# lambdaclass/simpleworks

Hardware: AMD Instinct MI355X
Metric: Marlin prove() constraints/sec at 2^20 R1CS; G1 MSM points/sec (higher is better)
Workload: dtype u32 limbs (384-bit Montgomery Fq for G1, 256-bit Fr); 1 GPU; marlin_prove: synthetic R1CS, 2^20 constraints = variables = non-zeros per matrix (|H| = |K| = 2^20), SRS + proving key device resident; per_gpu_units=1048576, multi_gpu=replicas (one proof per rank)

## Files before the change

simpleworks_amd/_lib.py:

```python
import contextlib
import ctypes
import json
import os

import numpy as np

_HERE = os.path.dirname(os.path.abspath(__file__))
LIB_PATH = os.environ.get("SWM_LIB_PATH") or os.path.join(_HERE, "libswmarlin.so")

_u64p = ctypes.POINTER(ctypes.c_uint64)
_u32p = ctypes.POINTER(ctypes.c_uint32)
_vp = ctypes.c_void_p
_sz = ctypes.c_size_t
_int = ctypes.c_int

ABI = {
    "swm_version": (_int, []),
    "swm_strerror": (ctypes.c_char_p, [_int]),
    "swm_init": (_int, [_int, ctypes.POINTER(_vp)]),
    "swm_destroy": (None, [_vp]),
    "swm_last_error": (ctypes.c_char_p, [_vp]),
    "swm_set_stream": (_int, [_vp, _vp]),
    "swm_set_msm_sharding": (_int, [_vp, ctypes.c_uint, ctypes.c_uint, _vp, _vp]),
    "swm_rccl_unique_id": (_int, [ctypes.c_void_p]),
# ... 1127 lines not shown
        self._check(self.lib.swm_blake2s_witness(self.h, a.ctypes.data if a.size else None, a.shape[1], a.shape[0], witness.ctypes.data,
                                                 digests.ctypes.data), "swm_blake2s_witness")
        return witness, digests

    def blake2s_witness_dev(self, d_inputs, input_len, count, d_witness, d_digests=None):
        self._check(self.lib.swm_blake2s_witness_dev(self.h, self._dev_ptr(d_inputs), input_len, count, self._dev_ptr(d_witness),
                                                     self._dev_ptr(d_digests)), "swm_blake2s_witness_dev")

    def profile_enable(self, on=True):
        self._check(self.lib.swm_profile_enable(self.h, int(on)), "swm_profile_enable")

    def profile_reset(self):
        self._check(self.lib.swm_profile_reset(self.h), "swm_profile_reset")

    def profile(self):
        buf = ctypes.create_string_buffer(1 << 20)
        self._check(self.lib.swm_profile_json(self.h, buf, len(buf)), "swm_profile_json")
        doc = json.loads(buf.value.decode())
        self.last_work = doc.get("work", {})
        self.last_calls = doc.get("calls", [])
        return {k["name"]: k for k in doc["kernels"]}

    def selftest_mul(self, which, a, b):
        a = np.ascontiguousarray(a, dtype=np.uint64)
        b = np.ascontiguousarray(b, dtype=np.uint64)
        out = np.empty_like(a)
        self._check(self.lib.swm_selftest_mul(self.h, which, _p64(a), _p64(b), _p64(out), a.shape[0]), "swm_selftest_mul")
        return out

    def selftest_g1_add(self, a_xy, b_xy):
        a = np.ascontiguousarray(a_xy, dtype=np.uint64).reshape(-1, 12)
        b = np.ascontiguousarray(b_xy, dtype=np.uint64).reshape(-1, 12)
        out = np.zeros((a.shape[0], 18), dtype=np.uint64)
        self._check(self.lib.swm_selftest_g1_add(self.h, _p64(a), _p64(b), _p64(out), a.shape[0]), "swm_selftest_g1_add")
        return out

    G1_CODEC_OPS = {"encode": 0, "decode": 1, "decode_unchecked": 2}

    def selftest_g1_codec(self, op, data, n):
        bad = ctypes.c_uint(0)
        if op == "encode":
            a = np.ascontiguousarray(data, dtype=np.uint64).reshape(n, 12)
            out = np.zeros(n * 96, dtype=np.uint8)
            self._check(self.lib.swm_selftest_g1_codec(self.h, 0, a.ctypes.data, n, out.ctypes.data, None), "swm_selftest_g1_codec")
            return out.tobytes()
        a = np.frombuffer(bytes(data), dtype=np.uint8).copy()
        assert a.size == n * 96
        out = np.zeros((n, 12), dtype=np.uint64)
        self._check(self.lib.swm_selftest_g1_codec(self.h, self.G1_CODEC_OPS[op], a.ctypes.data, n, out.ctypes.data, ctypes.byref(bad)),
                    "swm_selftest_g1_codec")
        return out, bad.value

    FR29_OPS = {"mul": 0, "mul_c": 1, "normalize": 2, "cond_sub_2r": 3, "cond_sub_r": 4, "canonical_below_2r": 5,
                "canonical": 6, "sub": 7, "unpack": 8, "pack": 9, "inv": 10, "inv_exact": 11}

    def selftest_fr29(self, op, a9, b9=None, spread9=None):
        a = np.ascontiguousarray(a9, dtype=np.uint32).reshape(-1, 9)
        b = np.ascontiguousarray(b9 if b9 is not None else a, dtype=np.uint32).reshape(-1, 9)
        assert b.shape == a.shape
        sp = np.ascontiguousarray(spread9 if spread9 is not None else np.zeros(9), dtype=np.uint32).reshape(9)
        out = np.zeros_like(a)
        self._check(self.lib.swm_selftest_fr29(self.h, self.FR29_OPS[op], _p32(a), _p32(b), _p32(sp), _p32(out), a.shape[0]),
                    "swm_selftest_fr29")
        return out

    P28_OPS = {"dbl": 0, "add": 1, "add_ool": 2, "slot_add": 3, "slot_add_inplace": 4, "slot_dbl": 5, "store_384": 6, "madd28": 7,
               "rows": 8, "te_from_row": 9, "te_madd_row": 10, "te_slot_add": 11, "te_slot_add_inplace": 12, "te_slot_add_self": 13,
               "te_slot_add_sync": 14, "te_store_384": 15, "quad_from_row": 16, "quad_madd_row": 17, "quad_add": 18,
               "quad_add_self": 19, "quad_store_identity": 20}

    def selftest_p28(self, op, a, b=None, flags=None, backmap=False, n=None):
        if a is not None:
            a = np.ascontiguousarray(a, dtype=np.uint64).reshape(-1, 12 if op == "rows" else 24)
            n = a.shape[0]
        if n is None:
            raise ValueError("selftest_p28: an op without operand a needs n")
        if b is not None:
            b = np.ascontiguousarray(b, dtype=np.uint64).reshape(-1, 24)
            assert b.shape[0] == n
        if flags is not None:
            flags = np.ascontiguousarray(flags, dtype=np.uint32).reshape(-1)
            assert flags.shape[0] == n
        out = np.zeros((n, 24), dtype=np.uint64)
        status = np.zeros(max(n, 1), dtype=np.uint32)
        jac = np.zeros((n, 18), dtype=np.uint64) if backmap else None
        self._check(self.lib.swm_selftest_p28(self.h, self.P28_OPS[op], _p64(a) if a is not None else None,
                                              _p64(b) if b is not None else None, _p32(flags) if flags is not None else None,
                                              _p64(out), _p64(jac) if backmap else None, _p32(status), n), "swm_selftest_p28")
        return out, status[:n], jac

    def _poly(self, op, data, n, m, z, pieces, out):
        zz = np.ascontiguousarray(z if z is not None else np.zeros(4), dtype=np.uint64).reshape(4)
        pc = np.ascontiguousarray(pieces if pieces is not None else np.zeros(2), dtype=np.uint64).reshape(-1)
        self._check(self.lib.swm_selftest_poly(self.h, op, data.ctypes.data, n, m, _p64(zz), _p64(pc), pc.size // 2,
                                               out.ctypes.data if out is not None else None), "swm_selftest_poly")

    def selftest_suffix_recurrence(self, a_mont, m, z_mont):
        a = np.ascontiguousarray(a_mont, dtype=np.uint64).reshape(-1, 4).copy()
        self._poly(0, a, a.shape[0], m, z_mont, None, None)
        return a

    def selftest_div_linear(self, p_mont, z_mont):
        p = np.ascontiguousarray(p_mont, dtype=np.uint64).reshape(-1, 4)
        out = np.zeros_like(p)
        self._poly(1, p, p.shape[0], 0, z_mont, None, out)
        return out

# ... 93 lines not shown
```

simpleworks_amd/csrc/capi.hip:

```cpp
#include <dlfcn.h>
#include <stdarg.h>
#include <string.h>
#include <algorithm>
#include <vector>
#include "context.h"
#include "g1.cuh"
#include "msm.h"

struct swm_rccl_id_arg {
    char internal[128];
};

namespace swm {

int ntt_run(swm_ctx* ctx, void* d_data, unsigned log_n, int inverse, int coset);
int ntt_sharded_run(swm_ctx* ctx, void* d_local, unsigned log_n, int inverse, int blocks_in);
struct SpmvPlan;
int spmv_run(swm_ctx* ctx, const void* d_rowptr, const void* d_col, const void* d_val, const void* d_z, void* d_out,
             size_t rows, const SpmvPlan* plan = nullptr);
int vec_mul_run(swm_ctx* ctx, const void* a, const void* b, void* out, size_t n);
int batch_inverse_run(swm_ctx* ctx, void* d, size_t n);
int selftest_mul_run(swm_ctx* ctx, int which, const void* a, const void* b, void* out, size_t n);
int selftest_chain_run(swm_ctx* ctx, int which, void* out, size_t threads, int iters);
int selftest_g1_add_run(swm_ctx* ctx, const void* a, const void* b, void* out, size_t n);
// ... 792 lines not shown
    snprintf(tail, sizeof(tail),
             "],\"work\":{\"msm_calls\":%llu,\"msm_points\":%llu,\"msm_digits\":%llu,\"msm_adds\":%llu,\"msm_zero_points\":%llu,\"msm_twins\":%llu,\"ntt_calls\":%llu,"
             "\"ntt_elements\":%llu,\"spmv_calls\":%llu,\"spmv_rows\":%llu,\"spmv_nnz\":%llu}}",
             (unsigned long long)ctx->stat_msm_calls, (unsigned long long)ctx->stat_msm_points,
             (unsigned long long)ctx->stat_msm_digits, (unsigned long long)ctx->stat_msm_adds,
             (unsigned long long)ctx->stat_msm_zero_points, (unsigned long long)ctx->stat_msm_twins, (unsigned long long)ctx->stat_ntt_calls, (unsigned long long)ctx->stat_ntt_elems,
             (unsigned long long)ctx->stat_spmv_calls, (unsigned long long)ctx->stat_spmv_rows,
             (unsigned long long)ctx->stat_spmv_nnz);
    s += tail;
    s.pop_back();
    s += ",\"calls\":[";
    for (size_t i = 0; i < ctx->call_log.size(); i++) {
        char item[48];
        snprintf(item, sizeof(item), "%s[\"%c\",%llu]", i ? "," : "", ctx->call_log[i].first,
                 (unsigned long long)ctx->call_log[i].second);
        s += item;
    }
    s += "]}";
    if (s.size() + 1 > buflen) return set_err(ctx, SWM_ERR_INVALID_ARG, "profile_json: buffer too small");
    memcpy(buf, s.c_str(), s.size() + 1);
    return SWM_OK;
}

int swm_selftest_witness_stage(swm_ctx* ctx, size_t bytes) {
    if (!ctx) return SWM_ERR_INVALID_ARG;
    ctx->witness_stage_bytes = bytes ? bytes : WITNESS_STAGE_BYTES;
    return SWM_OK;
}
int swm_selftest_exchange(swm_ctx* ctx, const void* d_send, void* d_recv, size_t bytes_per_peer, int alltoall) {
    if (!ctx || !d_send || !d_recv) return SWM_ERR_INVALID_ARG;
    SWM_ON_DEVICE(ctx);
    if (alltoall) SWM_TRY(shard_alltoall_dev(ctx, d_send, d_recv, bytes_per_peer));
    else SWM_TRY(shard_allgather_dev(ctx, d_send, bytes_per_peer, d_recv));
    SWM_HIP(ctx, hipStreamSynchronize(ctx->stream));
    return SWM_OK;
}
int swm_selftest_mul(swm_ctx* ctx, int which, const uint64_t* a, const uint64_t* b, uint64_t* out, size_t n) {
    if (!ctx || !a || !b || !out) return SWM_ERR_INVALID_ARG;
    SWM_ON_DEVICE(ctx);
    size_t es = which == 1 ? 32 : 48;
    char *da = nullptr, *db = nullptr;
    SWM_TRY(scratch(ctx, "stage.a", n * es + 64, (void**)&da));
    SWM_TRY(scratch(ctx, "stage.b", n * es + 64, (void**)&db));
    SWM_HIP(ctx, hipMemcpyAsync(da, a, n * es, hipMemcpyHostToDevice, ctx->stream));
    SWM_HIP(ctx, hipMemcpyAsync(db, b, n * es, hipMemcpyHostToDevice, ctx->stream));
    SWM_TRY(selftest_mul_run(ctx, which, da, db, da, n));
    SWM_HIP(ctx, hipMemcpyAsync(out, da, n * es, hipMemcpyDeviceToHost, ctx->stream));
    SWM_HIP(ctx, hipStreamSynchronize(ctx->stream));
    return SWM_OK;
}
int swm_selftest_fr29(swm_ctx* ctx, int op, const uint32_t* a9, const uint32_t* b9, const uint32_t* spread9, uint32_t* out9,
                      size_t n) {
    const bool two = op == 0 || op == 1 || op == 7;
    if (!ctx || op < 0 || op > 11 || (n && (!a9 || !out9 || (two && !b9))) || (op == 7 && !spread9)) return SWM_ERR_INVALID_ARG;
    SWM_ON_DEVICE(ctx);
    if (n == 0) return SWM_OK;
    const size_t bytes = n * 36;
    char *da = nullptr, *db = nullptr;
    SWM_TRY(scratch(ctx, "stage.a", bytes + 64, (void**)&da));
    SWM_TRY(scratch(ctx, "stage.b", bytes + 64, (void**)&db));
    SWM_HIP(ctx, hipMemcpyAsync(da, a9, bytes, hipMemcpyHostToDevice, ctx->stream));
    if (two) SWM_HIP(ctx, hipMemcpyAsync(db, b9, bytes, hipMemcpyHostToDevice, ctx->stream));
    SWM_TRY(selftest_fr29_run(ctx, op, da, db, op == 7 ? spread9 : nullptr, da, n));
    SWM_HIP(ctx, hipMemcpyAsync(out9, da, bytes, hipMemcpyDeviceToHost, ctx->stream));
    SWM_HIP(ctx, hipStreamSynchronize(ctx->stream));
    return SWM_OK;
}
int swm_selftest_p28(swm_ctx* ctx, int op, const uint64_t* a, const uint64_t* b, const uint32_t* flags, uint64_t* out, uint64_t* out_jac,
                     uint32_t* status, size_t n) {
    const bool rows = op == 8, te = (op >= 9 && op <= 14) || (op >= 16 && op <= 20);
    const bool two = op == 1 || op == 2 || op == 3 || op == 4 || op == 7 || op == 10 || op == 11 || op == 12 || op == 14 || op == 17 || op == 18;
    if (!ctx || op < 0 || op > 20 || (n && (!out || (op != 20 && !a) || (two && !b))) || (out_jac && !te)) return SWM_ERR_INVALID_ARG;
    SWM_ON_DEVICE(ctx);
    if (n == 0) return SWM_OK;
    const size_t in_bytes = n * (rows ? 96 : 192), out_bytes = n * 192;
    char *da = nullptr, *db = nullptr, *dc = nullptr, *dd = nullptr;
    SWM_TRY(scratch(ctx, "stage.a", out_bytes + 64, (void**)&da));
    SWM_TRY(scratch(ctx, "stage.b", out_bytes + 64, (void**)&db));
    SWM_TRY(scratch(ctx, "stage.c", out_bytes + 64, (void**)&dc));
    SWM_TRY(scratch(ctx, "stage.d", n * 200 + 64, (void**)&dd));
    char* d_pref = dd + n * 144;
    uint32_t *d_flags = (uint32_t*)(dd + n * 192), *d_status = d_flags + n;
    if (a) SWM_HIP(ctx, hipMemcpyAsync(da, a, in_bytes, hipMemcpyHostToDevice, ctx->stream));
    if (two) SWM_HIP(ctx, hipMemcpyAsync(db, b, out_bytes, hipMemcpyHostToDevice, ctx->stream));
    if (flags) SWM_HIP(ctx, hipMemcpyAsync(d_flags, flags, n * 4, hipMemcpyHostToDevice, ctx->stream));
    else SWM_HIP(ctx, hipMemsetAsync(d_flags, 0, n * 4, ctx->stream));
    SWM_HIP(ctx, hipMemsetAsync(d_status, 0, n * 4, ctx->stream));
    SWM_HIP(ctx, hipMemsetAsync(dc, 0xA5, out_bytes, ctx->stream));
    SWM_TRY(selftest_p28_run(ctx, op, da, db, d_flags, dc, out_jac ? dd : nullptr, d_pref, d_status, n));
    SWM_HIP(ctx, hipMemcpyAsync(out, dc, out_bytes, hipMemcpyDeviceToHost, ctx->stream));
    if (out_jac) SWM_HIP(ctx, hipMemcpyAsync(out_jac, dd, n * 144, hipMemcpyDeviceToHost, ctx->stream));
    if (status) SWM_HIP(ctx, hipMemcpyAsync(status, d_status, n * 4, hipMemcpyDeviceToHost, ctx->stream));
    SWM_HIP(ctx, hipStreamSynchronize(ctx->stream));
    return SWM_OK;
}
int swm_selftest_g1_add(swm_ctx* ctx, const uint64_t* a_xy, const uint64_t* b_xy, uint64_t* out_jac, size_t n) {
    if (!ctx || !a_xy || !b_xy || !out_jac) return SWM_ERR_INVALID_ARG;
    SWM_ON_DEVICE(ctx);
    char *da = nullptr, *db = nullptr, *dc = nullptr;
    SWM_TRY(scratch(ctx, "stage.a", n * 96 + 64, (void**)&da));
    SWM_TRY(scratch(ctx, "stage.b", n * 96 + 64, (void**)&db));
    SWM_TRY(scratch(ctx, "stage.c", n * 144 + 64, (void**)&dc));
    SWM_HIP(ctx, hipMemcpyAsync(da, a_xy, n * 96, hipMemcpyHostToDevice, ctx->stream));
    SWM_HIP(ctx, hipMemcpyAsync(db, b_xy, n * 96, hipMemcpyHostToDevice, ctx->stream));
    SWM_TRY(selftest_g1_add_run(ctx, da, db, dc, n));
    SWM_HIP(ctx, hipMemcpyAsync(out_jac, dc, n * 144, hipMemcpyDeviceToHost, ctx->stream));
    SWM_HIP(ctx, hipStreamSynchronize(ctx->stream));
// ... 109 lines not shown
```

simpleworks_amd/csrc/fr29.cuh:

```cuda
#pragma once
#include "ff.cuh"

namespace swm {

struct Fr29 {
    uint32_t l[9];
};
static constexpr uint32_t M29 = (1u << 29) - 1;
struct Fr29Consts {
    static constexpr uint32_t P[9] = SWM_FR29_P;
    static constexpr uint32_t ONE[9] = SWM_FR29_ONE;
    static constexpr uint32_t P2[9] = SWM_FR29_2P;
};

__device__ __forceinline__ Fr29 fr29_unpack(const Fr& a) {
    Fr29 r;
#pragma unroll
    for (int i = 0; i < 9; i++) {
        const int bit = 29 * i, w = bit >> 5, off = bit & 31;
        uint32_t v = a.v[w] >> off;
        if (off > 3 && w + 1 < 8) v |= a.v[w + 1] << (32 - off);
        r.l[i] = i < 8 ? (v & M29) : v;
    }
    return r;
// ... 33 lines not shown
#pragma unroll
    for (int i = 0; i < 9; i++) r.l[i] = a.l[i] + b.l[i];
    return r;
}
struct Spread29 {
    uint32_t l[9];
};
__device__ __forceinline__ Fr29 fr29_sub(const Fr29& a, const Fr29& b, const Spread29& sp) {
    Fr29 r;
#pragma unroll
    for (int i = 0; i < 9; i++) r.l[i] = a.l[i] + sp.l[i] - b.l[i];
    return r;
}
__device__ __forceinline__ Fr29 fr29_mul(const Fr29& a, const Fr29& b) {
    Fr29 r;
    uint32_t m[9];
    uint64_t acc = 0;
#pragma unroll
    for (int k = 0; k < 9; k++) {
#pragma unroll
        for (int i = 0; i <= k; i++) acc += (uint64_t)a.l[i] * b.l[k - i];
#pragma unroll
        for (int i = 0; i < k; i++) acc += (uint64_t)m[i] * Fr29Consts::P[k - i];
        m[k] = (0u - (uint32_t)acc) & M29;
        acc = (acc + m[k]) >> 29;
    }
#pragma unroll
    for (int k = 9; k < 17; k++) {
#pragma unroll
        for (int i = k - 8; i < 9; i++) acc += (uint64_t)a.l[i] * b.l[k - i];
#pragma unroll
        for (int i = k - 8; i < 9; i++) acc += (uint64_t)m[i] * Fr29Consts::P[k - i];
        r.l[k - 9] = (uint32_t)acc & M29;
        acc >>= 29;
    }
    r.l[8] = (uint32_t)acc;
    return r;
}
#include "fr29_mul_asm.inc"
__device__ __forceinline__ Fr29 fr29_mul_fenced(const Fr29& a, const Fr29& b) {
    Fr29 r;
    uint32_t m0, m1, m2, m3, m4, m5, m6, m7, m8;
    constexpr const uint32_t (&P)[9] = Fr29Consts::P;
    static_assert(P[0] == 1u, "the carry rule needs r = 1 mod 2^29");
    asm(SWM_FR29_MUL_ASM_TEXT
        : "=&v"(r.l[0]), "=&v"(r.l[1]), "=&v"(r.l[2]), "=&v"(r.l[3]), "=&v"(r.l[4]), "=&v"(r.l[5]), "=&v"(r.l[6]), "=&v"(r.l[7]),
          "=&v"(r.l[8]), "=&v"(m0), "=&v"(m1), "=&v"(m2), "=&v"(m3), "=&v"(m4), "=&v"(m5), "=&v"(m6), "=&v"(m7), "=&v"(m8)
        : "v"(a.l[0]), "v"(a.l[1]), "v"(a.l[2]), "v"(a.l[3]), "v"(a.l[4]), "v"(a.l[5]), "v"(a.l[6]), "v"(a.l[7]), "v"(a.l[8]),
          "v"(b.l[0]), "v"(b.l[1]), "v"(b.l[2]), "v"(b.l[3]), "v"(b.l[4]), "v"(b.l[5]), "v"(b.l[6]), "v"(b.l[7]), "v"(b.l[8]),
          "s"(P[1]), "s"(P[2]), "s"(P[3]), "s"(P[4]), "s"(P[5]), "s"(P[6]), "s"(P[7]), "s"(P[8]), "s"(M29), "s"((uint64_t)M29)
        : "v0", "v1", "vcc");
    return r;
}
__device__ __forceinline__ Fr29 fr29_cond_sub(const Fr29& a, const uint32_t (&k)[9]) {
    Fr29 t;
    uint32_t borrow = 0;
#pragma unroll
    for (int i = 0; i < 9; i++) {
        uint32_t d = a.l[i] - k[i] - borrow;
        borrow = d >> 31;
        t.l[i] = i < 8 ? (d & M29) : d;
    }
    Fr29 r;
#pragma unroll
    for (int i = 0; i < 9; i++) r.l[i] = borrow ? a.l[i] : t.l[i];
    return r;
}
__device__ __forceinline__ Fr29 fr29_canonical(const Fr29& a, bool below_2r) {
    Fr29 x = below_2r ? a : fr29_cond_sub(a, Fr29Consts::P2);
    return fr29_cond_sub(x, Fr29Consts::P);
}

}
```

simpleworks_amd/csrc/ntt.hip:

```cpp
#include <atomic>
#include "context.h"
#include "ff.cuh"
#include "fr29.cuh"
#include <string.h>
#include <algorithm>
#include <vector>

namespace swm {

static constexpr int NTT_THREADS = 256;
static constexpr unsigned NTT_MAX_LOG_R = 10;

struct NttPassArgs {
    const Fr* src;
    Fr* dst;
    unsigned log_n, log_r, log_ns;
    const Fr* tw_small;
    const Fr* tw_lo;
    const Fr* tw_hi;
    const Fr* cs_lo;
    const Fr* cs_hi;
    uint64_t src_len;
    const Fr* pass_tw;
    int coset_in;
// ... 155 lines not shown
    const NttPassArgs& a = args.a;
    const LazyPlan& P = args.plan;
    const unsigned R = 1u << a.log_r;
    const uint64_t n = 1ull << a.log_n;
    const uint64_t stride = n >> a.log_r;
    const uint64_t j0 = (uint64_t)blockIdx.x * J;
    const uint64_t ns_mask = (1ull << a.log_ns) - 1;
    const unsigned tw_shift = a.log_n - a.log_ns - a.log_r;
    const Fr* src = a.src + blockIdx.y * a.src_cstride;
    Fr* dst = a.dst + blockIdx.y * a.dst_cstride;
    const uint64_t cs_k = a.cos_k[blockIdx.y];
    for (unsigned e0 = 0; e0 < R * J; e0 += 4 * NTT_THREADS) {
        Fr xs[4];
#pragma unroll
        for (int u = 0; u < 4; u++) {
            unsigned e = e0 + threadIdx.x + u * NTT_THREADS;
            if (e < R * J) {
                const uint64_t at = j0 + e % J + (uint64_t)(e / J) * stride;
                xs[u] = at < a.src_len ? src[at] : fp_zero<Fr>();
                if (a.fold_in && at + n < a.src_len) xs[u] = fp_add(xs[u], fp_mul(a.fold[blockIdx.y], src[at + n]));
            }
        }
#pragma unroll
        for (int u = 0; u < 4; u++) {
            unsigned e = e0 + threadIdx.x + u * NTT_THREADS;
            if (e >= R * J) break;
            unsigned jj = e % J, t = e / J;
            uint64_t idx = j0 + jj + (uint64_t)t * stride;
            Fr29 x = fr29_unpack(xs[u]);
            if (a.coset_in) x = fr29_mul_fenced(x, two_level_pow29(a.cs_lo, a.cs_hi, idx * cs_k));
            if (a.log_ns != 0) {
                uint64_t k = (j0 + jj) & ns_mask;
                const Fr29 tw = a.pass_tw ? fr29_unpack(a.pass_tw[((uint64_t)t << a.log_ns) + k])
                                          : two_level_pow29(a.tw_lo, a.tw_hi, (k * t) << tw_shift);
                x = fr29_mul_fenced(x, tw);
            }
            tile_put(tile, t * J + jj, x);
        }
    }
    __syncthreads();
    unsigned h = R >> 1;
    if (a.log_r & 1) {
        for (unsigned bq = threadIdx.x; bq < (R >> 1) * J; bq += NTT_THREADS) {
            unsigned jj = bq % J, pos = bq / J;
            unsigned i0 = pos, i1 = i0 + h;
            Fr29 u = tile_get(tile, i0 * J + jj), v = tile_get(tile, i1 * J + jj);
            tile_put(tile, i0 * J + jj, fr29_normalize(fr29_add(u, v)));
            tile_put(tile, i1 * J + jj, fr29_mul_fenced(fr29_sub(u, v, P.r2), fr29_unpack(a.tw_small[pos])));
        }
        h >>= 1;
        __syncthreads();
    }
    unsigned step = 0;
    for (; h >= 2; h >>= 2, step++) {
        const unsigned hh = h >> 1, s1 = (R >> 1) / h, s2 = 2 * s1;
        const bool red = (P.reduce >> step) & 1u;
        const Spread29& S1 = P.s1[step];
        const Spread29& S2 = P.s2[step];
        for (unsigned q = threadIdx.x; q < (R >> 2) * J; q += NTT_THREADS) {
            unsigned jj = q % J, qq = q / J;
            unsigned p = qq & (hh - 1), blk = qq / hh;
            unsigned i0 = blk * 2 * h + p, i1 = i0 + hh, i2 = i0 + h, i3 = i2 + hh;
            Fr29 a0, a1, a2, a3;
            {
                Fr29 x0 = tile_get(tile, i0 * J + jj), x2 = tile_get(tile, i2 * J + jj);
                a0 = fr29_add(x0, x2);
                a2 = fr29_mul_fenced(fr29_sub(x0, x2, S1), fr29_unpack(a.tw_small[p * s1]));
            }
            {
                Fr29 x1 = tile_get(tile, i1 * J + jj), x3 = tile_get(tile, i3 * J + jj);
                a1 = fr29_add(x1, x3);
                a3 = fr29_mul_fenced(fr29_sub(x1, x3, S1), fr29_unpack(a.tw_small[(p + hh) * s1]));
            }
            const Fr29 w = fr29_unpack(a.tw_small[p * s2]);
            Fr29 y0 = fr29_add(a0, a1);
            y0 = red ? fr29_mul_fenced(y0, fr29_const(Fr29Consts::ONE)) : fr29_normalize(y0);
            tile_put(tile, i0 * J + jj, y0);
            tile_put(tile, i1 * J + jj, fr29_mul_fenced(fr29_sub(a0, a1, S2), w));
            tile_put(tile, i2 * J + jj, fr29_normalize(fr29_add(a2, a3)));
            tile_put(tile, i3 * J + jj, fr29_mul_fenced(fr29_sub(a2, a3, P.s4), w));
        }
        __syncthreads();
    }
    for (unsigned e = threadIdx.x; e < R * J; e += NTT_THREADS) {
        unsigned jj, u;
        if (a.log_ns == 0) {
            u = e % R;
            jj = e / R;
        } else {
            jj = e % J;
            u = e / J;
        }
        uint64_t j = j0 + jj;
        uint64_t k = j & ns_mask;
        uint64_t o = ((j - k) << a.log_r) + k + ((uint64_t)u << a.log_ns);
        Fr29 x = tile_get(tile, bitrev_u(u, a.log_r) * J + jj);
        if (a.scale_out) {
            Fr29 sc = fr29_unpack(a.n_inv);
            if (a.coset_out) sc = fr29_mul_fenced(two_level_pow29(a.cs_lo, a.cs_hi, o * cs_k), sc);
            x = fr29_canonical(fr29_mul_fenced(x, sc), true);
        } else if (args.last_pass) {
            x = fr29_canonical(x, P.out_below_2r != 0);
        }
        dst[o] = fr29_pack(x);
    }
}

static Fr host_root_of_unity(unsigned log_n, bool inverse) {
    Fr w;
    const uint32_t root[8] = SWM_FR_ROOT47_MONT;
    for (int i = 0; i < 8; i++) w.v[i] = root[i];
    for (unsigned i = log_n; i < 47; i++) w = fp_sqr(w);
    if (inverse) w = fp_inv(w);
    return w;
}

static int upload_powers(swm_ctx* ctx, const Fr& base, size_t count, void** out, bool lazy29 = false) {
    std::vector<Fr> h(count);
    Fr cur = lazy29 ? fp_from_u64<Fr>(32) : fp_one<Fr>();
    for (size_t i = 0; i < count; i++) {
        h[i] = cur;
        cur = fp_mul(cur, base);
    }
    SWM_HIP(ctx, hipMalloc(out, count * sizeof(Fr)));
    SWM_HIP(ctx, hipMemcpy(*out, h.data(), count * sizeof(Fr), hipMemcpyHostToDevice));
    return SWM_OK;
}

static int two_level_tables(swm_ctx* ctx, const Fr& base, size_t max_exp, NttTables* t, bool lazy29 = false) {
    SWM_TRY(upload_powers(ctx, base, 1024, &t->lo, lazy29));
    Fr b1024 = base;
    for (int i = 0; i < 10; i++) b1024 = fp_sqr(b1024);
    t->hi_len = (max_exp >> 10) + 1;
    SWM_TRY(upload_powers(ctx, b1024, t->hi_len, &t->hi, lazy29));
    return SWM_OK;
}
static constexpr uint64_t LAZY_KEY = 1ull << 50;

static int get_root_tables_form(swm_ctx* ctx, unsigned log_n, int inverse, bool lazy29, NttTables** out) {
    uint64_t key = ((uint64_t)log_n << 1) | (inverse ? 1 : 0) | (lazy29 ? LAZY_KEY : 0);
    auto it = ctx->ntt_tables.find(key);
    if (it == ctx->ntt_tables.end()) {
        NttTables t;
        SWM_TRY(two_level_tables(ctx, host_root_of_unity(log_n, inverse), 1ull << log_n, &t, lazy29));
        it = ctx->ntt_tables.emplace(key, t).first;
    }
    *out = &it->second;
    return SWM_OK;
}

int get_root_tables(swm_ctx* ctx, unsigned log_n, int inverse, NttTables** out) {
    return get_root_tables_form(ctx, log_n, inverse, false, out);
}

static int get_coset_tables(swm_ctx* ctx, unsigned log_n, int inverse, NttTables** out, bool lazy29 = false) {
    uint64_t key = (1ull << 40) | (inverse ? 1 : 0) | (lazy29 ? LAZY_KEY : 0);
    auto it = ctx->ntt_tables.find(key);
    if (it != ctx->ntt_tables.end() && it->second.hi_len < ((1ull << log_n) >> 10) + 1) {
        (void)hipFree(it->second.lo);
        (void)hipFree(it->second.hi);
        ctx->ntt_tables.erase(it);
        it = ctx->ntt_tables.end();
    }
    if (it == ctx->ntt_tables.end()) {
        Fr g;
        const uint32_t gm[8] = SWM_FR_GEN_MONT, gi[8] = SWM_FR_GEN_INV_MONT;
        for (int i = 0; i < 8; i++) g.v[i] = inverse ? gi[i] : gm[i];
        NttTables t;
        unsigned cap = log_n < 20 ? 20 : log_n;
        SWM_TRY(two_level_tables(ctx, g, 1ull << cap, &t, lazy29));
        it = ctx->ntt_tables.emplace(key, t).first;
    }
    *out = &it->second;
    return SWM_OK;
}

static int get_small_table(swm_ctx* ctx, unsigned log_r, int inverse, const Fr** out, bool lazy29 = false) {
    uint64_t key = ((uint64_t)log_r << 1) | (inverse ? 1 : 0) | (lazy29 ? LAZY_KEY : 0);
    auto it = ctx->ntt_small.find(key);
    if (it == ctx->ntt_small.end()) {
        void* d = nullptr;
        size_t cnt = log_r ? (1u << (log_r - 1)) : 1;
        SWM_TRY(upload_powers(ctx, host_root_of_unity(log_r, inverse), cnt, &d, lazy29));
        it = ctx->ntt_small.emplace(key, d).first;
    }
    *out = reinterpret_cast<const Fr*>(it->second);
    return SWM_OK;
}

__global__ void __launch_bounds__(256) ntt_build_pass_tw(const Fr* __restrict__ lo29, const Fr* __restrict__ hi29, unsigned log_ns,
                                                         unsigned log_r, unsigned shift, Fr* __restrict__ out) {
    const uint64_t x = blockIdx.x * (uint64_t)blockDim.x + threadIdx.x;
    if (x >> (log_ns + log_r)) return;
    const uint64_t k = x & (((uint64_t)1 << log_ns) - 1), t = x >> log_ns;
    out[x] = fr29_pack(fr29_canonical(two_level_pow29(lo29, hi29, (k * t) << shift), true));
}
static int get_pass_table(swm_ctx* ctx, unsigned log_n, int inverse, unsigned log_ns, unsigned log_r, const NttTables* rt29,
                          const Fr** out) {
    *out = nullptr;
    static const bool off = sw(SW_NTT_PASS_TABLES) == 0;
    if (off) return SWM_OK;
    const uint64_t key = (1ull << 51) | ((uint64_t)log_n << 20) | ((uint64_t)log_ns << 10) | ((uint64_t)log_r << 1) | (inverse ? 1 : 0);
    auto it = ctx->ntt_small.find(key);
    if (it == ctx->ntt_small.end()) {
        const size_t count = (size_t)1 << (log_ns + log_r);
        if (ctx->ntt_pass_table_bytes + count * sizeof(Fr) > ((size_t)4 << 30)) return SWM_OK;
        void* d = nullptr;
        if (hipMalloc(&d, count * sizeof(Fr)) != hipSuccess) {
            (void)hipGetLastError();
            return SWM_OK;
        }
        hipLaunchKernelGGL(ntt_build_pass_tw, dim3((unsigned)((count + 255) / 256)), dim3(256), 0, ctx->stream,
                           reinterpret_cast<const Fr*>(rt29->lo), reinterpret_cast<const Fr*>(rt29->hi), log_ns, log_r,
                           log_n - log_ns - log_r, reinterpret_cast<Fr*>(d));
        SWM_HIP(ctx, hipGetLastError());
        ctx->ntt_pass_table_bytes += count * sizeof(Fr);
        it = ctx->ntt_small.emplace(key, d).first;
    }
    *out = reinterpret_cast<const Fr*>(it->second);
    return SWM_OK;
}

static Spread29 lazy_spread(unsigned k, unsigned borrows) {
    Spread29 sp;
    uint64_t carry = 0;
    for (int i = 0; i < 9; i++) {
        uint64_t t = (uint64_t)Fr29Consts::P[i] * k + carry;
        sp.l[i] = i < 8 ? (uint32_t)(t & M29) : (uint32_t)t;
        carry = t >> 29;
    }
    sp.l[0] += borrows << 29;
    for (int i = 1; i < 8; i++) sp.l[i] += (borrows << 29) - borrows;
    sp.l[8] -= borrows;
    return sp;
}
static LazyPlan lazy_plan(unsigned log_r, unsigned b_in) {
    LazyPlan P;
    memset(&P, 0, sizeof(P));
    unsigned B = b_in;
    P.r2 = lazy_spread(2 * B, 1);
    if (log_r & 1) B = std::max(2 * B, 2u);
    const unsigned nsteps = log_r / 2;
    for (unsigned st = 0; st < nsteps && st < 6; st++) {
        P.s1[st] = lazy_spread(2 * B, 1);
        P.s2[st] = lazy_spread(4 * B, 2);
        const bool red = 4 * B > 64 || st + 1 == nsteps;
        if (red) P.reduce |= 1u << st;
        B = red ? 4 : 4 * B;
    }
    P.s4 = lazy_spread(4, 1);
    P.out_below_2r = B <= 2 ? 1u : 0u;
    return P;
}

int ntt_run_from(swm_ctx* ctx, void* d_data, unsigned log_n, int inverse, int coset, const void* first_src, size_t src_len);
int ntt_run(swm_ctx* ctx, void* d_data, unsigned log_n, int inverse, int coset) {
    return ntt_run_from(ctx, d_data, log_n, inverse, coset, nullptr, 0);
}
static int ntt_run_multi(swm_ctx* ctx, void* d_data, unsigned log_n, int inverse, int coset, const void* first_src, size_t src_len,
                         unsigned ncos, const unsigned* ks);
int ntt_run_from(swm_ctx* ctx, void* d_data, unsigned log_n, int inverse, int coset, const void* first_src, size_t src_len) {
    if (first_src && src_len > (1ull << std::min(log_n, 62u))) src_len = 1ull << log_n;
    return ntt_run_multi(ctx, d_data, log_n, inverse, coset ? 1 : 0, first_src, src_len, 1, nullptr);
}
int ntt_cosets_fwd(swm_ctx* ctx, const void* coeffs, size_t len, unsigned log_n, const unsigned* ks, unsigned ncos, void* out) {
    if (ncos < 1 || ncos > 4 || log_n > 28 || len > (2ull << log_n)) return set_err(ctx, SWM_ERR_INVALID_ARG, "ntt cosets: bad shape");
    for (unsigned c = 0; c < ncos; c++)
        if (ks[c] > 3) return set_err(ctx, SWM_ERR_INVALID_ARG, "ntt cosets: coset index > 3");
    return ntt_run_multi(ctx, out, log_n, 0, 2, coeffs, len, ncos, ks);
}
int ntt_cosets_inv(swm_ctx* ctx, void* data, unsigned log_n, unsigned ncos) {
    if (ncos < 1 || ncos > 4 || log_n > 28) return set_err(ctx, SWM_ERR_INVALID_ARG, "ntt cosets: bad shape");
    const unsigned ks[4] = {0, 1, 2, 3};
    return ntt_run_multi(ctx, data, log_n, 1, 2, nullptr, 0, ncos, ks);
}
static int ntt_run_multi(swm_ctx* ctx, void* d_data, unsigned log_n, int inverse, int coset, const void* first_src, size_t src_len,
                         unsigned ncos, const unsigned* ks) {
    if (log_n > 30) return set_err(ctx, SWM_ERR_INVALID_ARG, "ntt: log_n > 30 unsupported");
    const uint64_t n = 1ull << log_n;
    for (unsigned c = 0; c < ncos; c++) {
        ctx->stat_ntt_calls++;
        ctx->log_call('n', log_n);
        ctx->stat_ntt_elems += n;
    }
    Fr* data = reinterpret_cast<Fr*>(d_data);
    const uint64_t total = n * ncos;
    const unsigned maxr = NTT_MAX_LOG_R;
    static const bool lazy = sw(SW_NTT_LAZY) != 0;
    NttTables *rt = nullptr, *ct = nullptr;
    SWM_TRY(get_root_tables_form(ctx, log_n, inverse, lazy, &rt));
    if (coset == 1) SWM_TRY(get_coset_tables(ctx, log_n, inverse, &ct, lazy));
    if (coset == 2) SWM_TRY(get_root_tables_form(ctx, log_n + 2, inverse, lazy, &ct));
    Fr fold[4];
    for (unsigned c = 0; c < 4; c++) {
        fold[c] = fp_one<Fr>();
        if (coset == 2 && c < ncos)
            for (unsigned e = 0; e < ks[c]; e++) fold[c] = fp_mul(fold[c], host_root_of_unity(2, false));
    }
    Fr n_inv = fp_one<Fr>();
    if (inverse) n_inv = fp_inv(fp_from_u64<Fr>(n));
    if (lazy) n_inv = fp_mul(n_inv, fp_from_u64<Fr>(32));
    unsigned npass = log_n <= maxr ? 1 : (log_n + maxr - 1) / maxr;
    unsigned radices[8];
    {
        unsigned rem = log_n;
        for (unsigned p = 0; p < npass; p++) {
            unsigned r = (rem + (npass - p) - 1) / (npass - p);
            radices[p] = r;
            rem -= r;
        }
    }
    Fr *tmp = nullptr, *tmp2 = nullptr;
    SWM_TRY(scratch(ctx, "ntt.tmp", total * sizeof(Fr), (void**)&tmp));
    if (npass % 2 == 1 && npass >= 3) SWM_TRY(scratch(ctx, "ntt.tmp2", total * sizeof(Fr), (void**)&tmp2));
    const Fr* src = first_src ? reinterpret_cast<const Fr*>(first_src) : data;
    if (npass == 1 && !first_src) {
        SWM_HIP(ctx, hipMemcpyAsync(tmp, data, total * sizeof(Fr), hipMemcpyDeviceToDevice, ctx->stream));
        src = tmp;
    }
    unsigned log_ns = 0;
    for (unsigned p = 0; p < npass; p++) {
        NttPassArgs a;
        a.src = src;
        if (p == npass - 1) a.dst = data;
        else if (tmp2) a.dst = (p % 2 == 0) ? tmp : tmp2;
        else a.dst = (src == tmp) ? data : tmp;
        a.src_len = (p == 0 && first_src) ? (uint64_t)src_len : n;
        a.log_n = log_n;
        a.log_r = radices[p];
        a.log_ns = log_ns;
        SWM_TRY(get_small_table(ctx, a.log_r, inverse, &a.tw_small, lazy));
        a.tw_lo = reinterpret_cast<const Fr*>(rt->lo);
        a.tw_hi = reinterpret_cast<const Fr*>(rt->hi);
        a.cs_lo = ct ? reinterpret_cast<const Fr*>(ct->lo) : nullptr;
        a.cs_hi = ct ? reinterpret_cast<const Fr*>(ct->hi) : nullptr;
        a.pass_tw = nullptr;
        if (lazy && log_ns != 0) SWM_TRY(get_pass_table(ctx, log_n, inverse, log_ns, a.log_r, rt, &a.pass_tw));
        a.coset_in = (coset && !inverse && p == 0) ? 1 : 0;
        a.scale_out = (inverse && p == npass - 1) ? 1 : 0;
        a.coset_out = (coset && inverse && p == npass - 1) ? 1 : 0;
        a.n_inv = n_inv;
        a.src_cstride = (p == 0 && first_src) ? 0 : n;
        a.dst_cstride = n;
        a.fold_in = (coset == 2 && a.coset_in && src_len > n) ? 1 : 0;
        for (unsigned c = 0; c < 4; c++) {
            a.cos_k[c] = coset == 2 ? (c < ncos ? ks[c] : 0) : 1;
            a.fold[c] = fold[c];
        }
        uint64_t cols = n >> a.log_r;
        if (lazy) {
            NttLazyArgs la;
            la.a = a;
            la.plan = lazy_plan(a.log_r, (p > 0 || a.coset_in) ? 2u : 1u);
            la.last_pass = p == npass - 1 ? 1 : 0;
            unsigned J = 1;
            if (npass > 1) {
                J = (log_n >= 19 ? 1024u : 512u) >> a.log_r;
                if (J < 1) J = 1;
                if (J > 16) J = 16;
                while (J > cols) J >>= 1;
            }
            const size_t elems = (size_t)J << a.log_r;
            size_t shmem = (elems + (elems >> 5) + 1) * 36;
            if (shmem < 64) shmem = 64;
            dim3 grid((unsigned)(cols / J), ncos), block(NTT_THREADS);
            if (shmem > 64 * 1024) {
                static std::atomic<size_t> granted[64];
                if (J != 1 || shmem > 160 * 1024) return set_err(ctx, SWM_ERR_INVALID_ARG, "ntt: tile does not fit LDS");
                if (granted[ctx->device & 63].load() < shmem) {
                    SWM_HIP(ctx, hipFuncSetAttribute((const void*)ntt_pass_lazy<1>, hipFuncAttributeMaxDynamicSharedMemorySize, (int)shmem));
                    granted[ctx->device & 63].store(shmem);
                }
            }
            switch (J) {
                case 1: SWM_LAUNCH(ctx, "ntt_pass", ntt_pass_lazy<1>, grid, block, shmem, la); break;
                case 2: SWM_LAUNCH(ctx, "ntt_pass", ntt_pass_lazy<2>, grid, block, shmem, la); break;
                case 4: SWM_LAUNCH(ctx, "ntt_pass", ntt_pass_lazy<4>, grid, block, shmem, la); break;
                case 8: SWM_LAUNCH(ctx, "ntt_pass", ntt_pass_lazy<8>, grid, block, shmem, la); break;
                default: SWM_LAUNCH(ctx, "ntt_pass", ntt_pass_lazy<16>, grid, block, shmem, la); break;
            }
        } else if (npass == 1) {
            size_t shmem = sizeof(Fr) << a.log_r;
            if (shmem < 64) shmem = 64;
            SWM_LAUNCH(ctx, "ntt_pass", ntt_pass<1>, dim3((unsigned)cols, ncos), dim3(NTT_THREADS), shmem, a);
        } else {
            unsigned J = (log_n >= 19 ? 1024u : 512u) >> a.log_r;
            if (J < 1) J = 1;
            if (J > 16) J = 16;
            while (J > cols) J >>= 1;
            size_t shmem = (sizeof(Fr) * J) << a.log_r;
            dim3 grid((unsigned)(cols / J), ncos), block(NTT_THREADS);
            switch (J) {
// ... 86 lines not shown
```

simpleworks_amd/csrc/vec.hip:

```cpp
#include <string.h>
#include "context.h"
#include "fq28.cuh"
#include "fr29.cuh"
#include "frinv.cuh"
#include "g1.cuh"

namespace swm {

__global__ void __launch_bounds__(256) vec_mul_kernel(const Fr* __restrict__ a, const Fr* __restrict__ b,
                                                      Fr* __restrict__ out, size_t n) {
    SWM_LIGHT_KERNEL();
    for (size_t i = blockIdx.x * (size_t)blockDim.x + threadIdx.x; i < n; i += (size_t)gridDim.x * blockDim.x)
        out[i] = fp_mul(a[i], b[i]);
}

static constexpr int BINV_CHUNK = 16, BINV_CHUNK_SMALL = 4;
static constexpr int BINV_THREADS = 256;
template <int BINV_CHUNK>
__global__ void __launch_bounds__(BINV_THREADS) batch_inverse_kernel29(Fr* __restrict__ v, size_t n) {
    SWM_LIGHT_KERNEL();
    __shared__ Fr sp[BINV_THREADS], ss[BINV_THREADS];
    __shared__ Fr s_inv;
    const unsigned tid = threadIdx.x;
    size_t t = blockIdx.x * (size_t)blockDim.x + tid;
// ... 120 lines not shown
    b = a;
    b.x.l[1] ^= 0x1234;
    b.y.l[2] ^= (uint32_t)(i * 2654435761u) & 0xfff;
    for (int k = 0; k < iters; k++) {
        if (SITES == 1) {
            p28_add_fast<MulInline>(a, b);
        } else {
            p28_add_fast<MulInline>(a, b);
            p28_add_fast<MulInline>(b, a);
            p28_add_fast<MulInline>(a, b);
            p28_add_fast<MulInline>(b, a);
        }
    }
    out[i] = fq28_pack(fq28_canonical(fq28_mul(a.x, b.y)));
}
__global__ void __launch_bounds__(256) selftest_g1_add_kernel(const G1Affine* a, const G1Affine* b, G1Jac* out,
                                                              size_t n) {
    size_t i = blockIdx.x * (size_t)blockDim.x + threadIdx.x;
    if (i >= n) return;
    G1XYZZ acc = g1_from_affine(a[i]);
    g1_add_mixed(acc, b[i]);
    G1XYZZ twice = acc;
    g1_add(twice, acc);
    g1_add(twice, g1_neg(acc));
    out[i] = g1_to_jacobian(twice);
}

__global__ void __launch_bounds__(256) selftest_fr29_kernel(int op, const Fr29* a, const Fr29* b, Spread29 sp, Fr29* out, size_t n) {
    size_t i = blockIdx.x * (size_t)blockDim.x + threadIdx.x;
    if (i >= n) return;
    const Fr29 x = a[i];
    Fr w;
#pragma unroll
    for (int k = 0; k < 8; k++) w.v[k] = x.l[k];
    Fr29 r = fr29_const(Fr29Consts::P);
    auto words = [&](const Fr& v) {
#pragma unroll
        for (int k = 0; k < 8; k++) r.l[k] = v.v[k];
        r.l[8] = 0;
    };
    switch (op) {
        case 0: r = fr29_mul_fenced(x, b[i]); break;
        case 1: r = fr29_mul(x, b[i]); break;
        case 2: r = fr29_normalize(x); break;
        case 3: r = fr29_cond_sub(x, Fr29Consts::P2); break;
        case 4: r = fr29_cond_sub(x, Fr29Consts::P); break;
        case 5: r = fr29_canonical(x, true); break;
        case 6: r = fr29_canonical(x, false); break;
        case 7: r = fr29_sub(x, b[i], sp); break;
        case 8: r = fr29_unpack(w); break;
        case 9: words(fr29_pack(x)); break;
        case 10: words(fr_inv_single(w)); break;
        case 11: words(fr_inv_single_exact(w)); break;
        default: break;
    }
    out[i] = r;
}
int selftest_fr29_run(swm_ctx* ctx, int op, const void* a, const void* b, const uint32_t* sp9, void* out, size_t n) {
    if (n == 0) return SWM_OK;
    Spread29 sp;
    for (int k = 0; k < 9; k++) sp.l[k] = sp9 ? sp9[k] : 0u;
    SWM_LAUNCH(ctx, "selftest_fr29", selftest_fr29_kernel, dim3((unsigned)((n + 255) / 256)), dim3(256), 0, op, (const Fr29*)a,
               (const Fr29*)b, sp, (Fr29*)out, n);
    return SWM_OK;
}

int selftest_mul_run(swm_ctx* ctx, int which, const void* a, const void* b, void* out, size_t n) {
    unsigned grid = (unsigned)((n + 255) / 256);
    if (which == 6)
        SWM_LAUNCH(ctx, "selftest_mul2_28", selftest_mul2_28_kernel, dim3(grid), dim3(256), 0, (const Fq*)a, (const Fq*)b,
                   (Fq*)out, n);
    else if (which == 5)
        SWM_LAUNCH(ctx, "selftest_sqr28", selftest_sqr28_kernel, dim3(grid), dim3(256), 0, (const Fq*)a, (const Fq*)b,
                   (Fq*)out, n);
    else if (which == 2)
        SWM_LAUNCH(ctx, "selftest_mul28", selftest_mul28_kernel, dim3(grid), dim3(256), 0, (const Fq*)a, (const Fq*)b,
                   (Fq*)out, n);
    else if (which == 0)
        SWM_LAUNCH(ctx, "selftest_mul_fq", selftest_mul_kernel<Fq>, dim3(grid), dim3(256), 0, (const Fq*)a,
                   (const Fq*)b, (Fq*)out, n);
    else
        SWM_LAUNCH(ctx, "selftest_mul_fr", selftest_mul_kernel<Fr>, dim3(grid), dim3(256), 0, (const Fr*)a,
                   (const Fr*)b, (Fr*)out, n);
    return SWM_OK;
}
int selftest_chain_run(swm_ctx* ctx, int which, void* out, size_t threads, int iters) {
    unsigned grid = (unsigned)(threads / 256);
    if (which == 3)
        SWM_LAUNCH(ctx, "selftest_p28_1site", selftest_p28_add_chain<1>, dim3(grid), dim3(256), 0, (Fq*)out, iters);
    else if (which == 4)
        SWM_LAUNCH(ctx, "selftest_p28_4site", selftest_p28_add_chain<4>, dim3(grid), dim3(256), 0, (Fq*)out, iters / 4);
    else if (which == 2)
        SWM_LAUNCH(ctx, "selftest_chain28", selftest_mul28_chain, dim3(grid), dim3(256), 0, (Fq*)out, iters);
    else if (which == 0)
        SWM_LAUNCH(ctx, "selftest_chain_fq", selftest_mul_chain<Fq>, dim3(grid), dim3(256), 0, (Fq*)out, iters);
    else
        SWM_LAUNCH(ctx, "selftest_chain_fr", selftest_mul_chain<Fr>, dim3(grid), dim3(256), 0, (Fr*)out, iters);
    return SWM_OK;
}
int selftest_g1_add_run(swm_ctx* ctx, const void* a, const void* b, void* out, size_t n) {
    SWM_LAUNCH(ctx, "selftest_g1_add", selftest_g1_add_kernel, dim3((unsigned)((n + 255) / 256)), dim3(256), 0,
               (const G1Affine*)a, (const G1Affine*)b, (G1Jac*)out, n);
    return SWM_OK;
}

}
// ... 17 lines not shown
```

Before: 23.31 million constraints/s.

## Cheapen lazy NTT reductions, specialize final radix-2 stage, fold n^-1 into twiddles

Adds fr29_reduce, a quotient-estimate partial reduction that replaces the Montgomery multiply by one used to bound limb growth in the radix-4 NTT stages. The final h==2 stage gets its own radix-4 butterfly using a fixed twiddle. Inverse NTTs fold the n^-1 scale into the last pass's twiddle table or into a pre-scaled coset power table, which removes an extra multiply per output element. The reduction bounds change, so lazy-reduction correctness depends on the new spread and reduce plan being consistent.

```diff
diff --git a/simpleworks_amd/_lib.py b/simpleworks_amd/_lib.py
--- a/simpleworks_amd/_lib.py
+++ b/simpleworks_amd/_lib.py
@@ -1203,7 +1203,7 @@
         return out, bad.value
 
     FR29_OPS = {"mul": 0, "mul_c": 1, "normalize": 2, "cond_sub_2r": 3, "cond_sub_r": 4, "canonical_below_2r": 5,
-                "canonical": 6, "sub": 7, "unpack": 8, "pack": 9, "inv": 10, "inv_exact": 11}
+                "canonical": 6, "sub": 7, "unpack": 8, "pack": 9, "inv": 10, "inv_exact": 11, "reduce": 12}
 
     def selftest_fr29(self, op, a9, b9=None, spread9=None):
         a = np.ascontiguousarray(a9, dtype=np.uint32).reshape(-1, 9)
diff --git a/simpleworks_amd/csrc/capi.hip b/simpleworks_amd/csrc/capi.hip
--- a/simpleworks_amd/csrc/capi.hip
+++ b/simpleworks_amd/csrc/capi.hip
@@ -868,7 +868,7 @@
 int swm_selftest_fr29(swm_ctx* ctx, int op, const uint32_t* a9, const uint32_t* b9, const uint32_t* spread9, uint32_t* out9,
                       size_t n) {
     const bool two = op == 0 || op == 1 || op == 7;
-    if (!ctx || op < 0 || op > 11 || (n && (!a9 || !out9 || (two && !b9))) || (op == 7 && !spread9)) return SWM_ERR_INVALID_ARG;
+    if (!ctx || op < 0 || op > 12 || (n && (!a9 || !out9 || (two && !b9))) || (op == 7 && !spread9)) return SWM_ERR_INVALID_ARG;
     SWM_ON_DEVICE(ctx);
     if (n == 0) return SWM_OK;
     const size_t bytes = n * 36;
diff --git a/simpleworks_amd/csrc/fr29.cuh b/simpleworks_amd/csrc/fr29.cuh
--- a/simpleworks_amd/csrc/fr29.cuh
+++ b/simpleworks_amd/csrc/fr29.cuh
@@ -109,6 +109,24 @@
         : "v0", "v1", "vcc");
     return r;
 }
+__device__ __forceinline__ Fr29 fr29_reduce(const Fr29& a) {
+    constexpr const uint32_t (&P)[9] = Fr29Consts::P;
+    constexpr uint32_t RT1 = P[8] + 1;
+    constexpr uint32_t RECIP = (uint32_t)((1ull << 52) / RT1);
+    static_assert(((1ull << 52) / RT1) >> 32 == 0 && RT1 < (1u << 24), "the quotient estimate needs r_top + 1 between 2^20 and 2^24");
+    const uint32_t q = __umulhi(a.l[8] << 3, RECIP) >> 23;
+    Fr29 r;
+    uint32_t c = 0;
+#pragma unroll
+    for (int i = 0; i < 8; i++) {
+        const uint32_t ni = i == 0 ? M29 - P[0] + 1 : M29 - P[i];
+        const uint64_t acc = (uint64_t)q * ni + (uint32_t)(a.l[i] + c);
+        r.l[i] = (uint32_t)acc & M29;
+        c = (uint32_t)(acc >> 29);
+    }
+    r.l[8] = a.l[8] + c - __umul24(q, RT1);
+    return r;
+}
 __device__ __forceinline__ Fr29 fr29_cond_sub(const Fr29& a, const uint32_t (&k)[9]) {
     Fr29 t;
     uint32_t borrow = 0;
diff --git a/simpleworks_amd/csrc/ntt.hip b/simpleworks_amd/csrc/ntt.hip
--- a/simpleworks_amd/csrc/ntt.hip
+++ b/simpleworks_amd/csrc/ntt.hip
@@ -231,7 +231,7 @@
         __syncthreads();
     }
     unsigned step = 0;
-    for (; h >= 2; h >>= 2, step++) {
+    for (; h >= 4; h >>= 2, step++) {
         const unsigned hh = h >> 1, s1 = (R >> 1) / h, s2 = 2 * s1;
         const bool red = (P.reduce >> step) & 1u;
         const Spread29& S1 = P.s1[step];
@@ -253,11 +253,35 @@
             }
             const Fr29 w = fr29_unpack(a.tw_small[p * s2]);
             Fr29 y0 = fr29_add(a0, a1);
-            y0 = red ? fr29_mul_fenced(y0, fr29_const(Fr29Consts::ONE)) : fr29_normalize(y0);
+            y0 = red ? fr29_reduce(y0) : fr29_normalize(y0);
             tile_put(tile, i0 * J + jj, y0);
             tile_put(tile, i1 * J + jj, fr29_mul_fenced(fr29_sub(a0, a1, S2), w));
             tile_put(tile, i2 * J + jj, fr29_normalize(fr29_add(a2, a3)));
             tile_put(tile, i3 * J + jj, fr29_mul_fenced(fr29_sub(a2, a3, P.s4), w));
+        }
+        __syncthreads();
+    }
+    if (h == 2) {
+        const Spread29& S1 = P.s1[step];
+        const Spread29& S2 = P.s2[step];
+        const Fr29 w4 = fr29_unpack(a.tw_small[R >> 2]);
+        for (unsigned q = threadIdx.x; q < (R >> 2) * J; q += NTT_THREADS) {
+            const unsigned jj = q % J, i0 = (q / J) * 4;
+            Fr29 a0, a1, a2, a3;
+            {
+                Fr29 x0 = tile_get(tile, i0 * J + jj), x2 = tile_get(tile, (i0 + 2) * J + jj);
+                a0 = fr29_add(x0, x2);
+                a2 = fr29_sub(x0, x2, S1);
+            }
+            {
+                Fr29 x1 = tile_get(tile, (i0 + 1) * J + jj), x3 = tile_get(tile, (i0 + 3) * J + jj);
+                a1 = fr29_add(x1, x3);
+                a3 = fr29_mul_fenced(fr29_sub(x1, x3, S1), w4);
+            }
+            tile_put(tile, i0 * J + jj, fr29_reduce(fr29_add(a0, a1)));
+            tile_put(tile, (i0 + 1) * J + jj, fr29_reduce(fr29_sub(a0, a1, S2)));
+            tile_put(tile, (i0 + 2) * J + jj, fr29_reduce(fr29_add(a2, a3)));
+            tile_put(tile, (i0 + 3) * J + jj, fr29_reduce(fr29_sub(a2, a3, P.s4)));
         }
         __syncthreads();
     }
@@ -275,8 +299,7 @@
         uint64_t o = ((j - k) << a.log_r) + k + ((uint64_t)u << a.log_ns);
         Fr29 x = tile_get(tile, bitrev_u(u, a.log_r) * J + jj);
         if (a.scale_out) {
-            Fr29 sc = fr29_unpack(a.n_inv);
-            if (a.coset_out) sc = fr29_mul_fenced(two_level_pow29(a.cs_lo, a.cs_hi, o * cs_k), sc);
+            const Fr29 sc = a.coset_out ? two_level_pow29(a.cs_lo, a.cs_hi, o * cs_k) : fr29_unpack(a.n_inv);
             x = fr29_canonical(fr29_mul_fenced(x, sc), true);
         } else if (args.last_pass) {
             x = fr29_canonical(x, P.out_below_2r != 0);
@@ -294,9 +317,10 @@
     return w;
 }
 
-static int upload_powers(swm_ctx* ctx, const Fr& base, size_t count, void** out, bool lazy29 = false) {
+static int upload_powers(swm_ctx* ctx, const Fr& base, size_t count, void** out, bool lazy29 = false, const Fr* scale = nullptr) {
     std::vector<Fr> h(count);
     Fr cur = lazy29 ? fp_from_u64<Fr>(32) : fp_one<Fr>();
+    if (scale) cur = fp_mul(cur, *scale);
     for (size_t i = 0; i < count; i++) {
         h[i] = cur;
         cur = fp_mul(cur, base);
@@ -332,6 +356,12 @@
     return get_root_tables_form(ctx, log_n, inverse, false, out);
 }
 
+static Fr coset_generator(int inverse) {
+    Fr g;
+    const uint32_t gm[8] = SWM_FR_GEN_MONT, gi[8] = SWM_FR_GEN_INV_MONT;
+    for (int i = 0; i < 8; i++) g.v[i] = inverse ? gi[i] : gm[i];
+    return g;
+}
 static int get_coset_tables(swm_ctx* ctx, unsigned log_n, int inverse, NttTables** out, bool lazy29 = false) {
     uint64_t key = (1ull << 40) | (inverse ? 1 : 0) | (lazy29 ? LAZY_KEY : 0);
     auto it = ctx->ntt_tables.find(key);
@@ -342,15 +372,25 @@
         it = ctx->ntt_tables.end();
     }
     if (it == ctx->ntt_tables.end()) {
-        Fr g;
-        const uint32_t gm[8] = SWM_FR_GEN_MONT, gi[8] = SWM_FR_GEN_INV_MONT;
-        for (int i = 0; i < 8; i++) g.v[i] = inverse ? gi[i] : gm[i];
         NttTables t;
         unsigned cap = log_n < 20 ? 20 : log_n;
-        SWM_TRY(two_level_tables(ctx, g, 1ull << cap, &t, lazy29));
+        SWM_TRY(two_level_tables(ctx, coset_generator(inverse), 1ull << cap, &t, lazy29));
         it = ctx->ntt_tables.emplace(key, t).first;
     }
     *out = &it->second;
+    return SWM_OK;
+}
+
+static int get_scaled_coset_lo(swm_ctx* ctx, unsigned log_n, int coset, const Fr** out) {
+    const uint64_t key = (1ull << 52) | ((uint64_t)coset << 8) | log_n;
+    auto it = ctx->ntt_small.find(key);
+    if (it == ctx->ntt_small.end()) {
+        void* d = nullptr;
+        const Fr n_inv = fp_inv(fp_from_u64<Fr>(1ull << log_n));
+        SWM_TRY(upload_powers(ctx, coset == 1 ? coset_generator(1) : host_root_of_unity(log_n + 2, true), 1024, &d, true, &n_inv));
+        it = ctx->ntt_small.emplace(key, d).first;
+    }
+    *out = reinterpret_cast<const Fr*>(it->second);
     return SWM_OK;
 }
 
@@ -368,18 +408,21 @@
 }
 
 __global__ void __launch_bounds__(256) ntt_build_pass_tw(const Fr* __restrict__ lo29, const Fr* __restrict__ hi29, unsigned log_ns,
-                                                         unsigned log_r, unsigned shift, Fr* __restrict__ out) {
+                                                         unsigned log_r, unsigned shift, int scaled, Fr scale, Fr* __restrict__ out) {
     const uint64_t x = blockIdx.x * (uint64_t)blockDim.x + threadIdx.x;
     if (x >> (log_ns + log_r)) return;
     const uint64_t k = x & (((uint64_t)1 << log_ns) - 1), t = x >> log_ns;
-    out[x] = fr29_pack(fr29_canonical(two_level_pow29(lo29, hi29, (k * t) << shift), true));
+    Fr29 w = two_level_pow29(lo29, hi29, (k * t) << shift);
+    if (scaled) w = fr29_mul_fenced(w, fr29_unpack(scale));
+    out[x] = fr29_pack(fr29_canonical(w, true));
 }
 static int get_pass_table(swm_ctx* ctx, unsigned log_n, int inverse, unsigned log_ns, unsigned log_r, const NttTables* rt29,
-                          const Fr** out) {
+                          const Fr* scale29, const Fr** out) {
     *out = nullptr;
     static const bool off = sw(SW_NTT_PASS_TABLES) == 0;
     if (off) return SWM_OK;
-    const uint64_t key = (1ull << 51) | ((uint64_t)log_n << 20) | ((uint64_t)log_ns << 10) | ((uint64_t)log_r << 1) | (inverse ? 1 : 0);
+    const uint64_t key = (1ull << 51) | (scale29 ? 1ull << 53 : 0) | ((uint64_t)log_n << 20) | ((uint64_t)log_ns << 10) |
+                         ((uint64_t)log_r << 1) | (inverse ? 1 : 0);
     auto it = ctx->ntt_small.find(key);
     if (it == ctx->ntt_small.end()) {
         const size_t count = (size_t)1 << (log_ns + log_r);
@@ -391,7 +434,7 @@
         }
         hipLaunchKernelGGL(ntt_build_pass_tw, dim3((unsigned)((count + 255) / 256)), dim3(256), 0, ctx->stream,
                            reinterpret_cast<const Fr*>(rt29->lo), reinterpret_cast<const Fr*>(rt29->hi), log_ns, log_r,
-                           log_n - log_ns - log_r, reinterpret_cast<Fr*>(d));
+                           log_n - log_ns - log_r, scale29 ? 1 : 0, scale29 ? *scale29 : fp_one<Fr>(), reinterpret_cast<Fr*>(d));
         SWM_HIP(ctx, hipGetLastError());
         ctx->ntt_pass_table_bytes += count * sizeof(Fr);
         it = ctx->ntt_small.emplace(key, d).first;
@@ -423,7 +466,11 @@
     for (unsigned st = 0; st < nsteps && st < 6; st++) {
         P.s1[st] = lazy_spread(2 * B, 1);
         P.s2[st] = lazy_spread(4 * B, 2);
-        const bool red = 4 * B > 64 || st + 1 == nsteps;
+        if (st + 1 == nsteps) {
+            B = 2;
+            break;
+        }
+        const bool red = 4 * B > 64;
         if (red) P.reduce |= 1u << st;
         B = red ? 4 : 4 * B;
     }
@@ -479,6 +526,8 @@
     Fr n_inv = fp_one<Fr>();
     if (inverse) n_inv = fp_inv(fp_from_u64<Fr>(n));
     if (lazy) n_inv = fp_mul(n_inv, fp_from_u64<Fr>(32));
+    const Fr* cs_lo_scaled = nullptr;
+    if (lazy && coset && inverse) SWM_TRY(get_scaled_coset_lo(ctx, log_n, coset, &cs_lo_scaled));
     unsigned npass = log_n <= maxr ? 1 : (log_n + maxr - 1) / maxr;
     unsigned radices[8];
     {
@@ -511,12 +560,13 @@
         SWM_TRY(get_small_table(ctx, a.log_r, inverse, &a.tw_small, lazy));
         a.tw_lo = reinterpret_cast<const Fr*>(rt->lo);
         a.tw_hi = reinterpret_cast<const Fr*>(rt->hi);
-        a.cs_lo = ct ? reinterpret_cast<const Fr*>(ct->lo) : nullptr;
+        a.cs_lo = cs_lo_scaled ? cs_lo_scaled : ct ? reinterpret_cast<const Fr*>(ct->lo) : nullptr;
         a.cs_hi = ct ? reinterpret_cast<const Fr*>(ct->hi) : nullptr;
         a.pass_tw = nullptr;
-        if (lazy && log_ns != 0) SWM_TRY(get_pass_table(ctx, log_n, inverse, log_ns, a.log_r, rt, &a.pass_tw));
+        const bool fold_n_inv = lazy && inverse && !coset && log_ns != 0 && p == npass - 1;
+        if (lazy && log_ns != 0) SWM_TRY(get_pass_table(ctx, log_n, inverse, log_ns, a.log_r, rt, fold_n_inv ? &n_inv : nullptr, &a.pass_tw));
         a.coset_in = (coset && !inverse && p == 0) ? 1 : 0;
-        a.scale_out = (inverse && p == npass - 1) ? 1 : 0;
+        a.scale_out = (inverse && p == npass - 1 && !(fold_n_inv && a.pass_tw)) ? 1 : 0;
         a.coset_out = (coset && inverse && p == npass - 1) ? 1 : 0;
         a.n_inv = n_inv;
         a.src_cstride = (p == 0 && first_src) ? 0 : n;
diff --git a/simpleworks_amd/csrc/vec.hip b/simpleworks_amd/csrc/vec.hip
--- a/simpleworks_amd/csrc/vec.hip
+++ b/simpleworks_amd/csrc/vec.hip
@@ -196,6 +196,7 @@
         case 9: words(fr29_pack(x)); break;
         case 10: words(fr_inv_single(w)); break;
         case 11: words(fr_inv_single_exact(w)); break;
+        case 12: r = fr29_reduce(x); break;
         default: break;
     }
     out[i] = r;
```

New measurement: 23.50 million constraints/s (median of 6 runs). About the same (+0.8%).
